# ototoi/pbrt-r3

Hardware: AMD Instinct MI355X
Metric: Mrays/s (higher is better)
Workload: dtype f32

## Files before the change

pbrt-r3_amd/csrc/pt_kernels.hip:

```cpp
#include <hip/hip_runtime.h>
#include <cstdlib>
#include "pt_device.h"
#include "pt_device_math.h"
#include "pt_bxdf.h"
#include "pt_sphere.h"
#include "pt_quadric.h"
#include "pt_texture.h"
#include <type_traits>
#include "pt_lobes.h"
#include "pt_kernels.h"
#include "../../include/pbrtgpu.h"

#if PT_QUADRIC
#define PT_KERNEL __global__
#ifndef PT_KERNEL_NS
#define PT_KERNEL_NS ptq
#endif
namespace PT_KERNEL_NS {
#else
#define PT_KERNEL extern "C" __global__
#endif

#ifndef PT_LIGHTS_IN_LDS
#define PT_LIGHTS_IN_LDS 8
// ... 717 lines not shown
PT_DEV float v_max3(float a, float b, float c) { float r; asm("v_max3_f32 %0, %1, %2, %3" : "=v"(r) : "v"(a), "v"(b), "v"(c)); return r; }
PT_DEV float v_min3(float a, float b, float c) { float r; asm("v_min3_f32 %0, %1, %2, %3" : "=v"(r) : "v"(a), "v"(b), "v"(c)); return r; }

template <bool EXACT>
PT_DEV void visit_node_general(const PtNode* nodes, uint32_t ni, V3 o, V3 idir, uint32_t sbits, float tmin, float tmax, TravCtx& c, uint32_t& top, uint32_t& sa) {
    const char* nb = reinterpret_cast<const char*>(nodes) + (size_t)(ni & PT_REF_INDEX_MASK) * 128u;
    const uint32_t ox = (sbits & 1u) ? 48u : 0u, oy = (sbits & 2u) ? 48u : 0u, oz = (sbits & 4u) ? 48u : 0u;
    float4 nx = *reinterpret_cast<const float4*>(nb + ox), fx = *reinterpret_cast<const float4*>(nb + (48u - ox));
    float4 ny = *reinterpret_cast<const float4*>(nb + 16u + oy), fy = *reinterpret_cast<const float4*>(nb + 16u + (48u - oy));
    float4 nz = *reinterpret_cast<const float4*>(nb + 32u + oz), fz = *reinterpret_cast<const float4*>(nb + 32u + (48u - oz));
    uint4 ch = *reinterpret_cast<const uint4*>(nb + 96u);
    uint32_t axes = *reinterpret_cast<const uint32_t*>(nb + 112u);
    uint32_t mask = 0;
#define PT_SLAB(k, C)                                                        \
    {                                                                        \
        float a = tmin, b = tmax;                                            \
        if (EXACT) {                                                         \
            a = sse_max(a, (nx.C - o.x) * idir.x); b = sse_min(b, (fx.C - o.x) * idir.x); \
            a = sse_max(a, (ny.C - o.y) * idir.y); b = sse_min(b, (fy.C - o.y) * idir.y); \
            a = sse_max(a, (nz.C - o.z) * idir.z); b = sse_min(b, (fz.C - o.z) * idir.z); \
        } else {                                                             \
            a = fmaxf(a, (nx.C - o.x) * idir.x); b = fminf(b, (fx.C - o.x) * idir.x); \
            a = fmaxf(a, (ny.C - o.y) * idir.y); b = fminf(b, (fy.C - o.y) * idir.y); \
            a = fmaxf(a, (nz.C - o.z) * idir.z); b = fminf(b, (fz.C - o.z) * idir.z); \
        }                                                                    \
        if (b >= a) mask |= (1u << k);                                       \
    }
    PT_SLAB(0, x) PT_SLAB(1, y) PT_SLAB(2, z) PT_SLAB(3, w)
#undef PT_SLAB
    mask &= (axes >> 8) & 15u;
    uint32_t s_top = (sbits >> (axes & 3)) & 1, s_left = (sbits >> ((axes >> 2) & 3)) & 1, s_right = (sbits >> ((axes >> 4) & 3)) & 1;
    uint32_t l0 = s_left ? ch.x : ch.y, l1 = s_left ? ch.y : ch.x;
    uint32_t l0b = s_left ? 1u : 2u, l1b = s_left ? 2u : 1u;
    uint32_t r0 = s_right ? ch.z : ch.w, r1 = s_right ? ch.w : ch.z;
    uint32_t r0b = s_right ? 4u : 8u, r1b = s_right ? 8u : 4u;
    uint32_t c0 = s_top ? l0 : r0, c1 = s_top ? l1 : r1, c2 = s_top ? r0 : l0, c3 = s_top ? r1 : l1;
    uint32_t b0 = s_top ? l0b : r0b, b1 = s_top ? l1b : r1b, b2 = s_top ? r0b : l0b, b3 = s_top ? r1b : l1b;
    if (mask & b0) fs_push(c, sa, top, c0);
    if (mask & b1) fs_push(c, sa, top, c1);
    if (mask & b2) fs_push(c, sa, top, c2);
    if (mask & b3) fs_push(c, sa, top, c3);
}
PT_DEV void node_step_general(const PtScene& sc, LaneRay& r, TravCtx& c) {
    const uint32_t ref = fs_pop(c, r.sa, r.top);
    c.n_nodes++;
    if (r.sbits & 8u) visit_node_general<true>(sc.nodes, ref, r.o, r.idir, r.sbits, r.tmin, r.tmax, c, r.top, r.sa);
    else visit_node_general<false>(sc.nodes, ref, r.o, r.idir, r.sbits, r.tmin, r.tmax, c, r.top, r.sa);
}
PT_DEV void fs_push4_exec(uint32_t& sa, uint32_t& top, uint32_t c0, uint32_t c1, uint32_t c2, uint32_t c3, unsigned long long e0, unsigned long long e1,
                          unsigned long long e2, unsigned long long e3) {
    unsigned long long sv;
    asm volatile(
        "s_mov_b64 %[sv], exec\n\t"
        "s_mov_b64 exec, %[e0]\n\t"
        "v_add_u32 %[sa], %[slot], %[sa]\n\t"
        "v_mov_b32 %[top], %[c0]\n\t"
        "ds_write_b32 %[sa], %[c0]\n\t"
        "s_mov_b64 exec, %[e1]\n\t"
        "v_add_u32 %[sa], %[slot], %[sa]\n\t"
        "v_mov_b32 %[top], %[c1]\n\t"
        "ds_write_b32 %[sa], %[c1]\n\t"
        "s_mov_b64 exec, %[e2]\n\t"
        "v_add_u32 %[sa], %[slot], %[sa]\n\t"
        "v_mov_b32 %[top], %[c2]\n\t"
        "ds_write_b32 %[sa], %[c2]\n\t"
        "s_mov_b64 exec, %[e3]\n\t"
        "v_add_u32 %[sa], %[slot], %[sa]\n\t"
        "v_mov_b32 %[top], %[c3]\n\t"
        "ds_write_b32 %[sa], %[c3]\n\t"
        "s_mov_b64 exec, %[sv]"
        : [sa] "+v"(sa), [top] "+v"(top), [sv] "=&s"(sv)
        : [e0] "s"(e0), [e1] "s"(e1), [e2] "s"(e2), [e3] "s"(e3), [c0] "v"(c0), [c1] "v"(c1), [c2] "v"(c2), [c3] "v"(c3), [slot] "s"(PT_SLOT)
        : "memory");
}
typedef float pt_v4f __attribute__((ext_vector_type(4)));
typedef uint32_t pt_v4u __attribute__((ext_vector_type(4)));
PT_DEV float4 lds_load4(uint32_t a) { const pt_v4f v = *(__attribute__((address_space(3))) const pt_v4f*)(size_t)a; return make_float4(v.x, v.y, v.z, v.w); }
PT_DEV uint4 lds_load4u(uint32_t a) { const pt_v4u v = *(__attribute__((address_space(3))) const pt_v4u*)(size_t)a; return make_uint4(v.x, v.y, v.z, v.w); }
PT_DEV void node_step_lean(const PtScene& sc, LaneRay& r, TravCtx& c) {
    const uint32_t ref = r.top;
    r.sa -= PT_SLOT;
    uint32_t top = lds_load(r.sa);
    c.n_nodes++;
    const char* nb = reinterpret_cast<const char*>(sc.nodes);
    const uint32_t no = ref << 7;
    float4 nx, fx, ny, fy, nz, fz;
    uint4 ch;
#if PT_TOP_NODES > 0
    const bool in_lds = no < c.top_bytes;
    c.n_nodes_lds += in_lds ? 1u : 0u;
    if (in_lds) {
        const uint32_t la = c.top_lds + no - (no >> 3);
        nx = lds_load4(la + r.o_nx); fx = lds_load4(la + r.o_fx); ny = lds_load4(la + r.o_ny); fy = lds_load4(la + r.o_fy);
        nz = lds_load4(la + r.o_nz); fz = lds_load4(la + r.o_fz);
        ch = lds_load4u(la + 96u);
    }
    if (!in_lds)
#endif
    {
        nx = *reinterpret_cast<const float4*>(nb + (no + r.o_nx)); fx = *reinterpret_cast<const float4*>(nb + (no + r.o_fx));
        ny = *reinterpret_cast<const float4*>(nb + (no + r.o_ny)); fy = *reinterpret_cast<const float4*>(nb + (no + r.o_fy));
        nz = *reinterpret_cast<const float4*>(nb + (no + r.o_nz)); fz = *reinterpret_cast<const float4*>(nb + (no + r.o_fz));
        ch = *reinterpret_cast<const uint4*>(nb + (no + 96u));
    }
    const float ox = r.o.x, oy = r.o.y, oz = r.o.z, ix = r.idir.x, iy = r.idir.y, iz = r.idir.z;
#define PT_SLAB(C) (v_min3(v_min(r.tmax, (fx.C - ox) * ix), (fy.C - oy) * iy, (fz.C - oz) * iz) >= v_max3(v_max(r.tmin, (nx.C - ox) * ix), (ny.C - oy) * iy, (nz.C - oz) * iz))
    const bool h0 = PT_SLAB(x), h1 = PT_SLAB(y), h2 = PT_SLAB(z), h3 = PT_SLAB(w);
#undef PT_SLAB
    const bool T = __builtin_amdgcn_ubfe(r.sbits, __builtin_amdgcn_ubfe(ch.x, PT_REF_AXIS_SHIFT, 2), 1) != 0u;
    const bool L = __builtin_amdgcn_ubfe(r.sbits, __builtin_amdgcn_ubfe(ch.y, PT_REF_AXIS_SHIFT, 2), 1) != 0u;
    const bool R = __builtin_amdgcn_ubfe(r.sbits, __builtin_amdgcn_ubfe(ch.w, PT_REF_AXIS_SHIFT, 2), 1) != 0u;
    const uint32_t l0 = L ? ch.x : ch.y, l1 = L ? ch.y : ch.x, r0 = R ? ch.z : ch.w, r1 = R ? ch.w : ch.z;
    const uint32_t c0 = T ? l0 : r0, c1 = T ? l1 : r1, c2 = T ? r0 : l0, c3 = T ? r1 : l1;
    const unsigned long long H0 = __ballot(h0), H1 = __ballot(h1), H2 = __ballot(h2), H3 = __ballot(h3), Tm = __ballot(T), Lm = __ballot(L), Rm = __ballot(R);
    const unsigned long long yl = Lm & (H0 ^ H1), el0 = H1 ^ yl, el1 = H0 ^ yl;
    const unsigned long long yr = Rm & (H2 ^ H3), er0 = H3 ^ yr, er1 = H2 ^ yr;
    const unsigned long long y0 = Tm & (el0 ^ er0), e0 = er0 ^ y0, e2 = el0 ^ y0;
    const unsigned long long y1 = Tm & (el1 ^ er1), e1 = er1 ^ y1, e3 = el1 ^ y1;
    fs_push4_exec(r.sa, top, c0, c1, c2, c3, e0, e1, e2, e3);
    r.top = top;
}

#define PT_PAIR_U(x) ((uint32_t)__builtin_amdgcn_update_dpp(0, (int)(x), 0xB1, 0xF, 0xF, false))
#define PT_PAIR_F(x) __builtin_bit_cast(float, __builtin_amdgcn_update_dpp(0, __builtin_bit_cast(int, (x)), 0xB1, 0xF, 0xF, false))
PT_DEV void node_step_coop(const PtScene& sc, LaneRay& r, TravCtx& c, bool w_node, unsigned long long m_node) {
    constexpr unsigned long long kEven = 0x5555555555555555ull, kOdd = 0xAAAAAAAAAAAAAAAAull;
    const unsigned long long ev = m_node & kEven, od = m_node & kOdd;
    const unsigned long long m_y = ev | (ev << 1), m_z = od | (od >> 1);
    if (__builtin_amdgcn_inverse_ballot_w64(m_y | m_z)) {
        const uint32_t ref = r.top;
        const uint32_t no = ref << 7;
        const char* nb = reinterpret_cast<const char*>(sc.nodes);
        uint32_t top = PT_EMPTY_REF;
        const bool in_lds = w_node && no < c.top_bytes;
        if (w_node) { r.sa -= PT_SLOT; top = lds_load(r.sa); c.n_nodes++; c.n_nodes_lds += in_lds ? 1u : 0u; }
        const unsigned long long m_lds = __ballot(in_lds), le = m_lds & kEven, lo = m_lds & kOdd;
        const unsigned long long y_lds = le | (le << 1), z_lds = lo | (lo >> 1);
        const uint32_t base = in_lds ? c.top_lds + no - (no >> 3) : no;
        uint32_t a1 = base + r.o_nx, a2 = base + r.o_ny, a3 = base + r.o_nz;
        uint32_t b1 = PT_PAIR_U(base + r.o_fx), b2 = PT_PAIR_U(base + r.o_fy), b3 = PT_PAIR_U(base + r.o_fz);
        unsigned long long sv;
        asm volatile("s_mov_b64 %[sv], exec\n\ts_and_b64 exec, exec, %[om]\n\tv_swap_b32 %0, %3\n\tv_swap_b32 %1, %4\n\tv_swap_b32 %2, %5\n\ts_mov_b64 exec, %[sv]"
                     : "+v"(a1), "+v"(a2), "+v"(a3), "+v"(b1), "+v"(b2), "+v"(b3), [sv] "=&s"(sv) : [om] "s"(kOdd));
        float4 x1, x2, x3, x4, x5, x6;
        uint4 ch;
        if (__builtin_amdgcn_inverse_ballot_w64(m_y & y_lds)) { x1 = lds_load4(a1); x2 = lds_load4(a2); x3 = lds_load4(a3); }
        if (__builtin_amdgcn_inverse_ballot_w64(m_z & z_lds)) { x4 = lds_load4(b1); x5 = lds_load4(b2); x6 = lds_load4(b3); }
        if (in_lds) ch = lds_load4u(base + 96u);
        if (__builtin_amdgcn_inverse_ballot_w64(m_y & ~y_lds)) {
            x1 = *reinterpret_cast<const float4*>(nb + a1); x2 = *reinterpret_cast<const float4*>(nb + a2); x3 = *reinterpret_cast<const float4*>(nb + a3);
        }
        if (__builtin_amdgcn_inverse_ballot_w64(m_z & ~z_lds)) {
            x4 = *reinterpret_cast<const float4*>(nb + b1); x5 = *reinterpret_cast<const float4*>(nb + b2); x6 = *reinterpret_cast<const float4*>(nb + b3);
        }
        if (__builtin_amdgcn_inverse_ballot_w64(m_node & ~m_lds)) ch = *reinterpret_cast<const uint4*>(nb + (no + 96u));
        asm volatile("s_mov_b64 %[sv], exec\n\ts_and_b64 exec, exec, %[om]\n\t"
                     "v_swap_b32 %0, %12\n\tv_swap_b32 %1, %13\n\tv_swap_b32 %2, %14\n\tv_swap_b32 %3, %15\n\t"
                     "v_swap_b32 %4, %16\n\tv_swap_b32 %5, %17\n\tv_swap_b32 %6, %18\n\tv_swap_b32 %7, %19\n\t"
                     "v_swap_b32 %8, %20\n\tv_swap_b32 %9, %21\n\tv_swap_b32 %10, %22\n\tv_swap_b32 %11, %23\n\t"
                     "s_mov_b64 exec, %[sv]\n\ts_nop 1"
                     : "+v"(x1.x), "+v"(x1.y), "+v"(x1.z), "+v"(x1.w), "+v"(x2.x), "+v"(x2.y), "+v"(x2.z), "+v"(x2.w), "+v"(x3.x), "+v"(x3.y), "+v"(x3.z), "+v"(x3.w),
                       "+v"(x4.x), "+v"(x4.y), "+v"(x4.z), "+v"(x4.w), "+v"(x5.x), "+v"(x5.y), "+v"(x5.z), "+v"(x5.w), "+v"(x6.x), "+v"(x6.y), "+v"(x6.z), "+v"(x6.w), [sv] "=&s"(sv)
                     : [om] "s"(kOdd));
        const float ox = r.o.x, oy = r.o.y, oz = r.o.z, ix = r.idir.x, iy = r.idir.y, iz = r.idir.z;
#define PT_SLAB(C) (v_min3(v_min(r.tmax, (PT_PAIR_F(x4.C) - ox) * ix), (PT_PAIR_F(x5.C) - oy) * iy, (PT_PAIR_F(x6.C) - oz) * iz) >= \
                    v_max3(v_max(r.tmin, (x1.C - ox) * ix), (x2.C - oy) * iy, (x3.C - oz) * iz))
        const bool h0 = PT_SLAB(x), h1 = PT_SLAB(y), h2 = PT_SLAB(z), h3 = PT_SLAB(w);
#undef PT_SLAB
        const bool T = __builtin_amdgcn_ubfe(r.sbits, __builtin_amdgcn_ubfe(ch.x, PT_REF_AXIS_SHIFT, 2), 1) != 0u;
        const bool L = __builtin_amdgcn_ubfe(r.sbits, __builtin_amdgcn_ubfe(ch.y, PT_REF_AXIS_SHIFT, 2), 1) != 0u;
        const bool R = __builtin_amdgcn_ubfe(r.sbits, __builtin_amdgcn_ubfe(ch.w, PT_REF_AXIS_SHIFT, 2), 1) != 0u;
        const uint32_t l0 = L ? ch.x : ch.y, l1 = L ? ch.y : ch.x, r0 = R ? ch.z : ch.w, r1 = R ? ch.w : ch.z;
        const uint32_t c0 = T ? l0 : r0, c1 = T ? l1 : r1, c2 = T ? r0 : l0, c3 = T ? r1 : l1;
        const unsigned long long H0 = __ballot(h0) & m_node, H1 = __ballot(h1) & m_node, H2 = __ballot(h2) & m_node, H3 = __ballot(h3) & m_node;
        const unsigned long long Tm = __ballot(T), Lm = __ballot(L), Rm = __ballot(R);
        const unsigned long long yl = Lm & (H0 ^ H1), el0 = H1 ^ yl, el1 = H0 ^ yl;
        const unsigned long long yr = Rm & (H2 ^ H3), er0 = H3 ^ yr, er1 = H2 ^ yr;
        const unsigned long long y0 = Tm & (el0 ^ er0), e0 = er0 ^ y0, e2 = el0 ^ y0;
        const unsigned long long y1 = Tm & (el1 ^ er1), e1 = er1 ^ y1, e3 = el1 ^ y1;
        fs_push4_exec(r.sa, top, c0, c1, c2, c3, e0, e1, e2, e3);
        if (w_node) r.top = top;
    }
}

template <bool SPH, bool INST, bool ALPHA = false>
PT_DEV int32_t trace_closest(const PtScene& sc, V3 o, V3 d, float t_max, TravCtx& c, float* t_out, uint32_t* inst_out) {
// ... 48 lines not shown
        PREFETCH = 14, HANDOUT = 15,
        ITERATIONS = 16, HANDOUTS = 17, HANDOUTS_CLK = 18,
        EMPTY = 19, EMPTY_CLK = 20,
        SLOTS = 24
    };
    unsigned long long slot[SLOTS];
    long long t_start, t_iter, t_mark;
    bool handout;
    static PT_DEV long long now() { return (long long)__builtin_readcyclecounter(); }
    PT_DEV void start() { for (int i = 0; i < SLOTS; i++) slot[i] = 0; t_start = now(); }
    PT_DEV void iteration() {
        t_iter = now();
        handout = false;
        if ((slot[ITERATIONS]++ & 63ull) == 0ull) {
            const long long e0 = now();
            const long long e1 = now();
            slot[EMPTY] += 1; slot[EMPTY_CLK] += (unsigned long long)(e1 - e0);
            t_iter = now();
        }
        t_mark = t_iter;
    }
    PT_DEV void mark() { t_mark = now(); }
    PT_DEV void lap(int s) { const long long t = now(); slot[s] += (unsigned long long)(t - t_mark); t_mark = t; }
    PT_DEV void hand_out() { handout = true; }
    PT_DEV void handed_out() {
        const unsigned long long dt = (unsigned long long)(now() - t_mark);
        slot[HANDOUT] += dt;
        if (handout) { slot[HANDOUTS] += 1; slot[HANDOUTS_CLK] += dt; }
    }
    PT_DEV void serviced() { t_mark = now(); slot[SERVICE] += (unsigned long long)(t_mark - t_iter); }
    PT_DEV void round(int clk, int rounds, int items, unsigned long long n) { lap(clk); slot[rounds] += 1; slot[items] += n; }
    PT_DEV void node_round(unsigned long long lanes) { round(NODE, NODE_ROUNDS, NODE_LANES, (unsigned long long)__popcll(lanes)); }
    PT_DEV void general_round(unsigned long long lanes) { round(GENERAL, GENERAL_ROUNDS, NODE_LANES, (unsigned long long)__popcll(lanes)); }
    PT_DEV void leaf_round(unsigned long long items) { round(LEAF_FINISH, LEAF_ROUNDS, LEAF_ITEMS, items); }
    PT_DEV void leaf_issued() { lap(LEAF_ISSUE); asm volatile("s_waitcnt vmcnt(0)" ::: "memory"); lap(LEAF_WAIT); }
    PT_DEV void finish(uint32_t* diag, uint32_t lane) {
        slot[TOTAL] = (unsigned long long)(now() - t_start);
        if (lane == 0) for (int i = 0; i < SLOTS; i++) atomicAdd(reinterpret_cast<unsigned long long*>(diag) + i, slot[i]);
    }
};
#else
#define PT_PROF_BEGIN() ((void)0)
#define PT_PROF(call) ((void)0)
#endif
#ifndef PT_REFILL_MIN
#define PT_REFILL_MIN 8
#endif
#ifndef PT_LEAF_MIN
#define PT_LEAF_MIN 24
#endif
#ifndef PT_LEAF_MIN_INST
#define PT_LEAF_MIN_INST 40
#endif
#ifndef PT_TRACE_WAVES
#define PT_TRACE_WAVES 4
#endif
#ifndef PT_TRACE_DIST_WAVES
#define PT_TRACE_DIST_WAVES 4
#endif

#ifndef PT_LEAF_LANES_MIN
#define PT_LEAF_LANES_MIN 18
#endif
static_assert(PT_LEAF_LANES_MIN > 0, "the leaf round is triggered by the number of parked lanes");
#ifndef PT_SPH_LANES_MIN
#define PT_SPH_LANES_MIN 8
#endif
PT_DEV uint32_t wave_max_scan(uint32_t x) {
    x = max(x, (uint32_t)__builtin_amdgcn_update_dpp(0, (int)x, 0x111, 0xf, 0xf, false));
    x = max(x, (uint32_t)__builtin_amdgcn_update_dpp(0, (int)x, 0x112, 0xf, 0xf, false));
    x = max(x, (uint32_t)__builtin_amdgcn_update_dpp(0, (int)x, 0x114, 0xf, 0xf, false));
    x = max(x, (uint32_t)__builtin_amdgcn_update_dpp(0, (int)x, 0x118, 0xf, 0xf, false));
    x = max(x, (uint32_t)__builtin_amdgcn_update_dpp(0, (int)x, 0x142, 0xa, 0xf, false));
    x = max(x, (uint32_t)__builtin_amdgcn_update_dpp(0, (int)x, 0x143, 0xc, 0xf, false));
    return x;
}
template <bool DIST, bool SPH, bool INST = false, bool FAR = false, bool ALPHA = false>
PT_DEV void trace_body(const PtScene& sc, const PtPaths& P, const PtQueues& Q, PtCounters* cnt, uint32_t* spill, uint32_t spill_depth, uint32_t* err) {
    constexpr uint32_t TB = DIST ? PT_TBLOCK : PT_BLOCK;
    __shared__ uint32_t s_stack[(DIST ? PT_FS_SLOTS : PT_LDS_STACK) * TB];
    __shared__ unsigned long long s_cnt[4];
    __shared__ float4 s_res[DIST ? TB : 1];
#if PT_TOP_NODES > 0
    __shared__ float4 s_top[DIST ? PT_TOP_NODES * 7 : 1];
#endif
    TravCtx c;
    c.lds = &s_stack[threadIdx.x];
    c.top_lds = 0; c.top_bytes = 0; c.n_nodes_lds = 0;
    c.spill_stride = gridDim.x * TB;
    c.spill = spill + PT_DIAG_WORDS + (size_t)blockIdx.x * TB + threadIdx.x;
    c.spill_depth = spill_depth;
    c.n_nodes = 0; c.n_tris = 0; c.overflow = 0;
    c.lane_base = 0; c.stage_wave = 0; c.stage_own = 0; c.idx_pub = 0; c.idx_ld = 0;
    if constexpr (DIST) {
        s_stack[threadIdx.x] = PT_EMPTY_REF;
        c.lane_base = lds_addr_of(&s_stack[threadIdx.x]);
    }
#if PT_TOP_NODES > 0
    if constexpr (DIST) {
        const uint32_t n_top = min(sc.n_top, (uint32_t)PT_TOP_NODES);
        const float4* src = reinterpret_cast<const float4*>(sc.nodes);
        for (uint32_t k = threadIdx.x; k < n_top * 7u; k += TB) { const uint32_t nd = k / 7u; s_top[k] = src[nd * 8u + (k - nd * 7u)]; }
        c.top_lds = lds_addr_of(reinterpret_cast<const uint32_t*>(s_top));
        c.top_bytes = n_top << 7;
        __syncthreads();
    }
#endif
    const uint32_t n_cur = Q.counts[PT_Q_CUR], n_sh = Q.counts[PT_Q_SHADOW], n_pr = Q.counts[PT_Q_PROBE];
    const uint32_t total = n_cur + n_sh + n_pr;
    const uint32_t lane = threadIdx.x & 63;
    const unsigned long long below = (lane == 0) ? 0ull : (~0ull >> (64 - lane));
    unsigned long long regular = 0, shadow = 0;

    int kind = 0;
    uint32_t p = 0;
    LaneRay r;
    r.sp = 0;
    r.sa = c.lane_base; r.sa_limit = 0;
    r.top = PT_EMPTY_REF;
    bool more = total > 0;
    bool sph_wait = false;
    int pf_stage = 0, pf_kind = 0;
    uint32_t pf_raw = 0, pf_count = 0, pf_used = 0, pf_p = 0;
    uint32_t seg = blockIdx.x & 7u, seg_dry = 0;
    const uint32_t seg_len = (((total + 7u) >> 3) + 63u) & ~63u;
    float4 pf_o = make_float4(0.0f, 0.0f, 0.0f, 0.0f), pf_d = pf_o;
    PT_PROF_BEGIN();
    for (;;) {
        PT_PROF(iteration());
        constexpr bool PF_BYPASS = DIST && !FAR;
        int pf_gate = pf_stage;
        if constexpr (PF_BYPASS) asm volatile("" : "+s"(pf_gate));
        if (PF_BYPASS && pf_gate == 3) {
        } else if (pf_stage == 0) {
            if (more) {
                if (lane == 0) pf_raw = atomicAdd(&Q.counts[PT_Q_SEG_TICKET0 + 32u * seg], 64u);
                pf_stage = 1;
            }
        } else if (pf_stage == 1) {
            const uint32_t seg_lo = seg * seg_len, seg_hi = min(total, seg_lo + seg_len);
            const uint32_t base = seg_lo + (uint32_t)__builtin_amdgcn_readfirstlane((int)pf_raw);
            if (seg_lo >= total || base >= seg_hi) {
                seg = (seg + 1u) & 7u;
                if (++seg_dry == 8u) more = false;
                pf_stage = 0;
            } else {
                seg_dry = 0;
                pf_count = min(64u, seg_hi - base);
                pf_used = 0;
                const uint32_t item = base + lane;
                if (lane < pf_count) {
                    if (item < n_cur) { pf_p = Q.cur[item]; pf_kind = 1; }
                    else if (item < n_cur + n_sh) { pf_p = Q.shadow[item - n_cur]; pf_kind = 2; }
                    else { pf_p = Q.probe[item - n_cur - n_sh]; pf_kind = 3; }
                }
                pf_stage = 2;
            }
        } else if (pf_stage == 2) {
            if (lane < pf_count) {
                const float4* so = pf_kind == 1 ? P.ray_o : (pf_kind == 2 ? P.sh_o : P.pr_o);
                const float4* sd = pf_kind == 1 ? P.ray_d : (pf_kind == 2 ? P.sh_d : P.pr_d);
                pf_o = so[pf_p]; pf_d = sd[pf_p];
            }
            pf_stage = 3;
        }
        PT_PROF(lap(PhaseProf::PREFETCH));
        constexpr bool LATE_RETIRE = DIST;
#define PT_RETIRE()                                                                                                                                      \
        if (kind != 0 && ray_done(r)) {                                                                                                                  \
            if (kind == 1) { P.hit_t[p] = r.ray_tmax; P.hit_rec[p] = r.best; if (INST && (!ALPHA || sc.n_instances)) P.hit_inst[p] = r.best_inst; }      \
            else if (kind == 2) P.occluded[p] = r.best >= 0 ? 1 : 0;                                                                                     \
            else P.probe_rec[p] = r.best;                                                                                                                \
            kind = 0;                                                                                                                                    \
        }
        if constexpr (LATE_RETIRE) {
            if (!more) { PT_RETIRE() }
        } else {
            PT_RETIRE()
        }
        {
            const unsigned long long idle = LATE_RETIRE ? __ballot(kind == 0 || ray_done(r)) : __ballot(kind == 0);
            const uint32_t n_idle = (uint32_t)__popcll(idle);
            if (pf_stage == 3 && (n_idle >= PT_REFILL_MIN || idle == ~0ull || (!more && n_idle != 0))) {
                PT_PROF(hand_out());
                if constexpr (LATE_RETIRE) { PT_RETIRE() }
                const uint32_t take = min(n_idle, pf_count - pf_used);
                const uint32_t rank = (uint32_t)__popcll(idle & below);
                const int src = (int)((pf_used + rank) & 63u);
                const uint32_t np = (uint32_t)__shfl((int)pf_p, src, 64);
                const int nk = __shfl(pf_kind, src, 64);
                float4 ro, rd;
                ro.x = __shfl(pf_o.x, src, 64); ro.y = __shfl(pf_o.y, src, 64); ro.z = __shfl(pf_o.z, src, 64); ro.w = __shfl(pf_o.w, src, 64);
                rd.x = __shfl(pf_d.x, src, 64); rd.y = __shfl(pf_d.y, src, 64); rd.z = __shfl(pf_d.z, src, 64);
                if (kind == 0 && rank < take) {
                    p = np; kind = nk;
                    if (nk == 2) shadow++; else regular++;
                    if constexpr (DIST) ray_begin_fs(sc, r, c, f4_3(ro), mk3(rd.x, rd.y, rd.z), ro.w);
                    else ray_begin(sc, r, f4_3(ro), mk3(rd.x, rd.y, rd.z), ro.w);
                }
                pf_used += take;
                if (pf_used == pf_count) pf_stage = 0;
            }
        }
#undef PT_RETIRE
        PT_PROF(handed_out());
        if ((LATE_RETIRE ? __ballot(kind != 0 && !ray_done(r)) : __ballot(kind != 0)) == 0) {
            if (!more && pf_stage == 0) break;
            continue;
        }
        bool w_tri = kind != 0 && ray_wants_tri(r);
        bool w_node = kind != 0 && ray_wants_node(r);
        unsigned long long m_tri = __ballot(w_tri), m_node = __ballot(w_node);
        PT_PROF(serviced());
        if constexpr (DIST) {
            bool sround = false;
            unsigned long long m_tri_s = 0;
            if constexpr (SPH) {
                m_tri_s = __ballot(w_tri && sph_wait);
                m_tri &= ~m_tri_s;
            }
            const bool sph_go = SPH && (uint32_t)__popcll(m_tri_s) >= (uint32_t)PT_SPH_LANES_MIN;
            const uint32_t tcnt = w_tri ? ((r.top >> PT_LEAF_COUNT_SHIFT) & 7u) + 1u : 0u;
            uint32_t tcnt_r = tcnt;
            bool w_serve = w_tri;
            constexpr uint32_t LEAF_DUE = 56u;
            unsigned long long c0 = 0, c1 = 0, c2 = 0, c3 = 0;
            const uint32_t leaf_level = (sph_go || (uint32_t)__popcll(m_tri) >= (uint32_t)PT_LEAF_LANES_MIN) ? LEAF_DUE : 0u;
            const uint32_t wbase = threadIdx.x & ~63u;
            constexpr bool HACC = !SPH;
            uint32_t lf_pre = 0, lf_items = 0;
            bool lf_served = false, lf_valid = false;
            int lf_kk = 0;
            float lf_tmax = PT_INF;
            RayPre lf_rp;
            TriVerts lf_tv;
            auto leaf_issue = [&](auto sr_tag) {
                constexpr bool SR = decltype(sr_tag)::value;
                (void)SR;
                c0 = __ballot((tcnt_r & 1u) != 0); c1 = __ballot((tcnt_r & 2u) != 0); c2 = __ballot((tcnt_r & 4u) != 0); c3 = __ballot((tcnt_r & 8u) != 0);
                lf_pre = (uint32_t)(__popcll(c0 & below) + 2 * __popcll(c1 & below) + 4 * __popcll(c2 & below) + 8 * __popcll(c3 & below));
                lf_served = w_serve && lf_pre + tcnt_r <= 64u;
                const unsigned long long m_served = __ballot(lf_served);
                const int last = 63 - __clzll(m_served);
                lf_items = (uint32_t)__shfl((int)(lf_pre + tcnt_r), last, 64);
                typedef uint32_t __attribute__((may_alias)) map_word;
                map_word* const s_own = reinterpret_cast<map_word*>(&s_res[wbase]);
                s_own[lane] = 0u;
                if (lf_served) s_own[lf_pre] = ((lf_pre << 6) | lane) + 1u;
                __builtin_amdgcn_fence(__ATOMIC_RELEASE, "wavefront");
                __builtin_amdgcn_wave_barrier();
                __builtin_amdgcn_fence(__ATOMIC_ACQUIRE, "wavefront");
                lf_valid = lane < lf_items;
                const uint32_t own_w = wave_max_scan(s_own[lane]) - 1u;
                const int o = (int)(own_w & 63u);
                const uint32_t k = lane - (own_w >> 6);
                const uint32_t first = (uint32_t)__shfl((int)(r.top & PT_LEAF_FIRST_MASK), o, 64);
                lf_rp.o = mk3(__shfl(r.rp.o.x, o, 64), __shfl(r.rp.o.y, o, 64), __shfl(r.rp.o.z, o, 64));
                lf_rp.d = mk3(0.0f, 0.0f, 0.0f);
                if ((SPH && SR) || sc.any_one_sided) lf_rp.d = mk3(__shfl(r.rp.d.x, o, 64), __shfl(r.rp.d.y, o, 64), __shfl(r.rp.d.z, o, 64));
                if constexpr ((SPH && SR) || HACC) lf_tmax = __shfl(r.ray_tmax, o, 64);
                lf_kk = __shfl(r.rp.kx | (r.rp.ky << 2) | (r.rp.kz << 4) | ((kind == 2 ? 1 : 0) << 6), o, 64);
                lf_rp.kx = lf_kk & 3; lf_rp.ky = (lf_kk >> 2) & 3; lf_rp.kz = (lf_kk >> 4) & 3;
                lf_rp.sx = __shfl(r.rp.sx, o, 64); lf_rp.sy = __shfl(r.rp.sy, o, 64); lf_rp.sz = __shfl(r.rp.sz, o, 64);
                lf_rp.dperm = lf_rp.d;
                lf_tv.p0 = lf_rp.d; lf_tv.p1 = lf_rp.d; lf_tv.p2 = lf_rp.d; lf_tv.prim = 0; lf_tv.flags = 0;
                if (lf_valid) lf_tv = load_tri(sc.tris, first + k);
            };
            auto leaf_finish = [&](auto sr_tag) {
                constexpr bool SR = decltype(sr_tag)::value;
                (void)SR;
                bool sphere_rec = false;
                if constexpr (SPH) sphere_rec = lf_valid && (lf_tv.flags & PT_TRI_SPHERE) != 0;
                unsigned long long m_sitems = 0;
                if constexpr (SPH && !SR) { m_sitems = __ballot(sphere_rec); }
                bool cand = false;
                if (lf_valid) {
                    asm("" : "+v"(lf_tv.p0.x), "+v"(lf_tv.p0.y), "+v"(lf_tv.p0.z), "+v"(lf_tv.p1.x), "+v"(lf_tv.p1.y), "+v"(lf_tv.p1.z), "+v"(lf_tv.p2.x), "+v"(lf_tv.p2.y), "+v"(lf_tv.p2.z));
                    TriCore tc;
                    const bool tri_ok = tri_core(lf_rp, lf_tv.p0, lf_tv.p1, lf_tv.p2, lf_tv.flags, tc);
                    float4 res = make_float4(tri_ok ? 1.0f : 0.0f, tc.t_scaled, tc.det, tc.t);
                    if constexpr (HACC) cand = tri_ok && tri_accept(tc.t_scaled, tc.det, lf_tmax);
                    if (SR && sphere_rec) {
                        SphHit sh;
                        sh.t = 0.0f; sh.a_hi = 0.0f; sh.b_hi = 0.0f;
                        const bool ok = shape_hit_test_inl(sc.spheres[__float_as_uint(lf_tv.p0.x)], lf_rp.o, lf_rp.d, lf_tmax, (lf_kk & 64) ? 2.0f * PT_PI : PT_PI, &sh);
                        res = make_float4(ok ? 2.0f : 0.0f, sh.a_hi, sh.b_hi, sh.t);
                        cand = ok;
                    }
                    if (!HACC || cand) s_res[wbase + lane] = res;
                }
                const unsigned long long m_cand = HACC ? __ballot(cand) : 0ull;
                (void)m_cand;
                __builtin_amdgcn_fence(__ATOMIC_RELEASE, "wavefront");
                __builtin_amdgcn_wave_barrier();
                __builtin_amdgcn_fence(__ATOMIC_ACQUIRE, "wavefront");
                bool walk = lf_served;
                if constexpr (SPH) {
                    if (!SR && lf_served && ((m_sitems >> lf_pre) & ((1ull << tcnt_r) - 1ull)) != 0ull) { sph_wait = true; walk = false; }
                    if (SR && lf_served) sph_wait = false;
                }
                if (walk) {
                    const uint32_t rec0 = fs_pop(c, r.sa, r.top) & PT_LEAF_FIRST_MASK;
                    const bool any_hit = kind == 2;
                    bool leaf_hit = false;
                    uint32_t tested = tcnt;
                    if constexpr (HACC) {
                    uint32_t bits = (uint32_t)(m_cand >> lf_pre) & ((1u << tcnt) - 1u);
                    bool first = true;
                    while (bits != 0u) {
                        const uint32_t k = (uint32_t)__builtin_ctz(bits);
                        bits &= bits - 1u;
                        const float4 v = s_res[wbase + lf_pre + k];
                        bool acc;
                        if (SPH && SR && v.x == 2.0f) acc = !(v.y > r.ray_tmax) && !(v.z > r.ray_tmax);
                        else acc = first || tri_accept(v.y, v.z, r.ray_tmax);
                        first = false;
                        if (acc) {
                            r.best = (int32_t)(rec0 + k); leaf_hit = true;
                            if (any_hit) { r.sa = c.lane_base; r.top = PT_EMPTY_REF; tested = k + 1u; break; }
                            r.ray_tmax = v.w;
                        }
                    }
                    } else {
                    bool stop = false;
                    for (uint32_t k0 = 0; k0 < tcnt && !stop; k0 += 4u) {
                        const uint32_t b = wbase + lf_pre + k0;
                        const float4 va = s_res[b], vb = s_res[wbase + min(lf_pre + k0 + 1u, 63u)], vc = s_res[wbase + min(lf_pre + k0 + 2u, 63u)],
                                     vd = s_res[wbase + min(lf_pre + k0 + 3u, 63u)];
                        auto step = [&](const float4 v, uint32_t k) {
                            if (stop || k >= tcnt) return;
                            bool acc;
                            if (SPH && SR && v.x == 2.0f) acc = !(v.y > r.ray_tmax) && !(v.z > r.ray_tmax);
                            else acc = v.x != 0.0f && tri_accept(v.y, v.z, r.ray_tmax);
                            if (acc) {
                                r.best = (int32_t)(rec0 + k); leaf_hit = true;
                                if (any_hit) { r.sa = c.lane_base; r.top = PT_EMPTY_REF; tested = k + 1; stop = true; return; }
                                r.ray_tmax = v.w;
                            }
                        };
                        step(va, k0); step(vb, k0 + 1u); step(vc, k0 + 2u); step(vd, k0 + 3u);
                    }
                    }
                    c.n_tris += tested;
                    if (leaf_hit && !any_hit) r.tmax = r.ray_tmax;
                }
            };
            const bool lean = __ballot(w_node && r.sa >= r.sa_limit) == 0ull;
            if (lean && m_node != 0 && leaf_level < LEAF_DUE) {
                PT_PROF(mark());
                if constexpr (FAR) node_step_coop(sc, r, c, w_node, m_node);
                else if (w_node) node_step_lean(sc, r, c);
                PT_PROF(node_round(m_node));
            } else if (m_node != 0 && leaf_level < LEAF_DUE) {
                PT_PROF(mark());
                if (w_node) node_step_general(sc, r, c);
                PT_PROF(general_round(m_node));
            } else if ((m_tri | m_tri_s) != 0) {
                if constexpr (SPH) {
                    sround = sph_go || m_tri == 0;
                    w_serve = w_tri && (sph_wait == sround);
                    tcnt_r = w_serve ? tcnt : 0u;
                }
                PT_PROF(mark());
                if (SPH && sround) leaf_issue(std::true_type{}); else leaf_issue(std::false_type{});
                PT_PROF(leaf_issued());
                if (SPH && sround) leaf_finish(std::true_type{}); else leaf_finish(std::false_type{});
                PT_PROF(leaf_round(lf_items));
            }
        } else {
        if (m_node != 0 && __popcll(m_tri) < (INST ? PT_LEAF_MIN_INST : PT_LEAF_MIN)) {
            if (w_node) ray_step_node(sc, r, c);
            PT_PROF(general_round(m_node));
        } else {
            if constexpr (INST) {
                if (w_tri) {
                    if (r.top == PT_INST_EXIT_REF) {
                        (void)stk_pop(c, r.top, r.sp);
                        const float w_tmax = __uint_as_float(stk_pop(c, r.top, r.sp)), w_tmin = __uint_as_float(stk_pop(c, r.top, r.sp));
                        const float4 ro = (kind == 1 ? P.ray_o : (kind == 2 ? P.sh_o : P.pr_o))[p], rd = (kind == 1 ? P.ray_d : (kind == 2 ? P.sh_d : P.pr_d))[p];
                        const bool hit_inside = r.best >= 0 && r.best_inst == r.cur_inst;
                        ray_set_direction_state(r, f4_3(ro), mk3(rd.x, rd.y, rd.z));
                        r.tmin = w_tmin; r.tmax = hit_inside ? r.ray_tmax : w_tmax;
                        r.cur_inst = 0;
                    } else ray_step_tri_enter<SPH, ALPHA>(sc, r, kind == 2, c);
                }
            } else {
                if (w_tri) ray_step_tri<SPH, INST>(sc, r, kind == 2, c);
            }
            PT_PROF(leaf_round((unsigned long long)__popcll(m_tri)));
        }
        }
    }
    PT_PROF(finish(spill, lane));
    if (c.overflow) atomicOr(err, 1u);
    flush_counters(cnt, s_cnt, regular, shadow, c.n_nodes, c.n_tris);
    {
        unsigned long long v = c.n_nodes_lds;
        for (int o = 32; o > 0; o >>= 1) v += (unsigned long long)__shfl_xor((int)(v >> 32), o, 64) << 32 | (unsigned int)__shfl_xor((int)(unsigned int)v, o, 64);
        if ((threadIdx.x & 63) == 0 && v) atomicAdd(&cnt->nodes_lds, v);
    }
}
PT_KERNEL void __launch_bounds__(PT_TBLOCK, PT_TRACE_DIST_WAVES) k_trace(PtScene sc, PtPaths P, PtQueues Q, PtCounters* cnt, uint32_t* spill,
                                                              uint32_t spill_depth, uint32_t* err) {
    trace_body<true, false>(sc, P, Q, cnt, spill, spill_depth, err);
}
PT_KERNEL void __launch_bounds__(PT_TBLOCK, PT_TRACE_DIST_WAVES) k_trace_far(PtScene sc, PtPaths P, PtQueues Q, PtCounters* cnt, uint32_t* spill,
                                                                   uint32_t spill_depth, uint32_t* err) {
    trace_body<true, false, false, true>(sc, P, Q, cnt, spill, spill_depth, err);
}
PT_KERNEL void __launch_bounds__(PT_BLOCK, PT_TRACE_WAVES) k_trace_seq(PtScene sc, PtPaths P, PtQueues Q, PtCounters* cnt, uint32_t* spill,
                                                                  uint32_t spill_depth, uint32_t* err) {
    trace_body<false, false>(sc, P, Q, cnt, spill, spill_depth, err);
}
#ifndef PT_TRACE_INST_WAVES
#define PT_TRACE_INST_WAVES 3
#endif

PT_KERNEL void __launch_bounds__(PT_BLOCK, PT_TRACE_INST_WAVES) k_trace_inst(PtScene sc, PtPaths P, PtQueues Q, PtCounters* cnt, uint32_t* spill,
                                                                       uint32_t spill_depth, uint32_t* err) {
    trace_body<false, true, true>(sc, P, Q, cnt, spill, spill_depth, err);
}
PT_KERNEL void __launch_bounds__(PT_BLOCK, PT_TRACE_INST_WAVES) k_trace_alpha(PtScene sc, PtPaths P, PtQueues Q, PtCounters* cnt, uint32_t* spill,
                                                                        uint32_t spill_depth, uint32_t* err) {
    trace_body<false, true, true, false, true>(sc, P, Q, cnt, spill, spill_depth, err);
}
PT_KERNEL void __launch_bounds__(PT_TBLOCK, PT_TRACE_DIST_WAVES) k_trace_sph_dist(PtScene sc, PtPaths P, PtQueues Q, PtCounters* cnt, uint32_t* spill,
                                                                           uint32_t spill_depth, uint32_t* err) {
    trace_body<true, true>(sc, P, Q, cnt, spill, spill_depth, err);
}
PT_KERNEL void __launch_bounds__(PT_BLOCK, 2) k_trace_sph(PtScene sc, PtPaths P, PtQueues Q, PtCounters* cnt, uint32_t* spill,
// ... 2998 lines not shown
```

pbrt-r3_amd/csrc/pt_scene_upload.cpp:

```cpp
#include "pt_context_impl.h"

namespace {

bool load_sobol(pt_context* ctx) {
    std::string path = ctx->data_dir + "/sobol_tables.bin";
    FILE* f = std::fopen(path.c_str(), "rb");
    if (!f) return false;
    char magic[8];
    uint32_t hdr[4];
    bool ok = std::fread(magic, 1, 8, f) == 8 && std::memcmp(magic, "PTSOBOL1", 8) == 0 && std::fread(hdr, 4, 4, f) == 4;
    if (ok) {
        ctx->sobol_msize = hdr[1];
        ctx->sobol_n_vdc = hdr[2];
        ctx->sobol_n_inv = hdr[3];
        ctx->sobol_m32.resize((size_t)hdr[0] * hdr[1]);
        ctx->sobol_vdc.resize((size_t)hdr[2] * hdr[1]);
        ctx->sobol_inv.resize((size_t)hdr[3] * hdr[1]);
        ok = std::fread(ctx->sobol_m32.data(), 4, ctx->sobol_m32.size(), f) == ctx->sobol_m32.size() &&
             std::fread(ctx->sobol_vdc.data(), 8, ctx->sobol_vdc.size(), f) == ctx->sobol_vdc.size() &&
             std::fread(ctx->sobol_inv.data(), 8, ctx->sobol_inv.size(), f) == ctx->sobol_inv.size();
    }
    std::fclose(f);
    return ok;
}
// ... 1149 lines not shown
    return PT_OK;
}

pt_status upload_images_and_textures(pt_context* ctx, const pt_scene_desc* d, const SceneChecks& chk, const MaterialTables& mt, bool& images_on_device) {
    pt_status st;
    std::vector<PtImage> dimages(d->n_images);
    images_on_device =(mt.any_textured || !ctx->inf_lights.empty() || !ctx->map_lights.empty() || mt.any_alpha_tex) && d->n_images;
    if (images_on_device) {
        size_t total = 0;
        for (uint32_t i = 0; i < d->n_images; i++) {
            const pt_image& im = d->images[i];
            PtImage& o = dimages[i];
            std::memset(&o, 0, sizeof(o));
            o.width = im.width; o.height = im.height; o.channels = im.channels; o.n_levels = im.n_levels;
            uint32_t w = im.width, h = im.height;
            size_t off = 0;
            for (uint32_t l = 0; l < im.n_levels; l++) {
                if (off > 0xffffffffull) return ctx->fail(PT_ERR_UNSUPPORTED, "image pyramid larger than 2^32 floats");
                o.level_off[l] = (uint32_t)off;
                off += (size_t)w * h * im.channels;
                if (w > 1) w /= 2;
                if (h > 1) h /= 2;
            }
            total += off;
        }
        std::vector<float> all(total);
        size_t at = 0;
        std::vector<size_t> base(d->n_images);
        for (uint32_t i = 0; i < d->n_images; i++) {
            size_t n = 0;
            uint32_t w = d->images[i].width, h = d->images[i].height;
            for (uint32_t l = 0; l < d->images[i].n_levels; l++) { n += (size_t)w * h * d->images[i].channels; if (w > 1) w /= 2; if (h > 1) h /= 2; }
            std::memcpy(all.data() + at, d->images[i].texels, n * sizeof(float));
            base[i] = at;
            at += n;
        }
        if ((st = upload(ctx, ctx->d_image_texels, all.data(), all.size())) != PT_OK) return st;
        for (uint32_t i = 0; i < d->n_images; i++) dimages[i].texels = ctx->d_image_texels.as<float>() + base[i];
        if ((st = upload(ctx, ctx->d_images, dimages.data(), dimages.size())) != PT_OK) return st;
    } else { ctx->d_image_texels.release(); ctx->d_images.release(); }
    if (mt.any_textured || chk.any_alpha) {
        if (d->n_textures) { if ((st = upload(ctx, ctx->d_textures, d->textures, d->n_textures)) != PT_OK) return st; } else ctx->d_textures.release();
        if ((st = upload(ctx, ctx->d_tex_prog, mt.tex_prog.data(), mt.tex_prog.size())) != PT_OK) return st;
    } else { ctx->d_textures.release(); ctx->d_tex_prog.release(); }
    if (mt.any_textured) { if ((st = upload(ctx, ctx->d_mat_params, mt.mparams.data(), mt.mparams.size())) != PT_OK) return st; } else ctx->d_mat_params.release();
    if (d->N) { if ((st = upload(ctx, ctx->d_N, d->N, 3 * (size_t)d->n_vertices)) != PT_OK) return st; } else ctx->d_N.release();
    if (d->S) { if ((st = upload(ctx, ctx->d_S, d->S, 3 * (size_t)d->n_vertices)) != PT_OK) return st; } else ctx->d_S.release();
    if (d->UV) { if ((st = upload(ctx, ctx->d_UV, d->UV, 2 * (size_t)d->n_vertices)) != PT_OK) return st; } else ctx->d_UV.release();
    return PT_OK;
}

void fill_scene_record(pt_context* ctx, const pt_scene_desc* d, const SceneChecks& chk, const MaterialTables& mt, const WorldBuild& w, bool images_on_device) {
    PtScene& sc = ctx->sc;
    sc.nodes = ctx->d_nodes.as<PtNode>();
    sc.tris = ctx->d_tris.as<PtTri>();
    sc.tri_info = ctx->d_tri_info.as<PtTriInfo>();
    sc.N = d->N ? ctx->d_N.as<float>() : nullptr;
    sc.S = d->S ? ctx->d_S.as<float>() : nullptr;
    sc.UV = d->UV ? ctx->d_UV.as<float>() : nullptr;
    sc.materials = ctx->d_materials.as<PtMaterial>();
    sc.general_materials = mt.general_materials ? 1u : 0u;
    ctx->scene_has_lobe_materials = mt.general_materials;
    sc.any_one_sided = w.any_one_sided ? 1u : 0u;
    sc.dist_leaves = (w.up_max_leaf <= 8 && !std::getenv("PBRTGPU_SEQ_LEAVES")) ? 1u : 0u;
    ctx->n_materials = d->n_materials;
    sc.lights = ctx->d_lights.as<PtLight>();
    sc.n_lights = (uint32_t)w.lights.size();
    sc.textured = mt.any_textured ? 1u : 0u;
    sc.textures = (mt.any_textured || chk.any_alpha) && d->n_textures ? ctx->d_textures.as<pt_texture>() : nullptr;
    sc.tex_prog = (mt.any_textured || chk.any_alpha) ? ctx->d_tex_prog.as<uint32_t>() : nullptr;
    ctx->scene_alpha = chk.any_alpha;
    ctx->quadric_kernels = false;
    for (uint32_t i = 0; i < d->n_spheres; i++) ctx->quadric_kernels |= d->spheres[i].kind != PT_SHAPE_SPHERE;
    sc.images = images_on_device ? ctx->d_images.as<PtImage>() : nullptr;
    sc.mat_params = mt.any_textured ? ctx->d_mat_params.as<PtMatParams>() : nullptr;
    sc.spheres = d->n_spheres ? ctx->d_spheres.as<PtSphere>() : nullptr;
    sc.instances = d->n_instances ? ctx->d_instances.as<PtInstance>() : nullptr;
    sc.n_instances = d->n_instances;
    sc.n_spheres = d->n_spheres;
    if (d->n_spheres) sc.general_materials = 1;
    if (d->n_instances) { sc.general_materials = 1; sc.dist_leaves = 0; }
    sc.general_materials = (sc.general_materials & 1u) | ((uint32_t)mt.mixes.size() << 1);
    sc.root_ref = w.up_root_ref;
    sc.n_top = w.n_top;
    for (int a = 0; a < 3; a++) { const float ext = w.up_root_hi[a] - w.up_root_lo[a]; sc.cell_scale[a] = ext > 0.0f ? (float)(1u << PT_SORT_CELL_BITS) / ext : 0.0f; }
    std::memcpy(sc.wb_min, w.up_root_lo, 12);
    std::memcpy(sc.wb_max, w.up_root_hi, 12);
}

pt_status build_delta_and_env_records(pt_context* ctx, const pt_scene_desc* d, const std::vector<PtLight>& lights, std::vector<float>& env_power, std::vector<float>& delta_power) {
    PtScene& sc = ctx->sc;
    pt_status st;
    env_power.assign(ctx->inf_lights.size(), 0.0f);
    delta_power.assign(ctx->delta_lights.size() + ctx->map_lights.size(), 0.0f);
    sc.n_envs = 0;
    sc.n_deltas = 0;
    std::vector<PtEnvLight> envs(ctx->inf_lights.size());
    std::vector<PtDeltaLight> deltas(ctx->delta_lights.size() + ctx->map_lights.size());
    std::vector<PtMapLight> maps(ctx->map_lights.size());
    ctx->maplight_kernels = !ctx->map_lights.empty();
    const float dx = sc.wb_max[0] - sc.wb_min[0], dy = sc.wb_max[1] - sc.wb_min[1], dz = sc.wb_max[2] - sc.wb_min[2];
    const float radius = std::sqrt(dx * dx + dy * dy + dz * dz) * 0.5f;
    if (!ctx->delta_lights.empty()) {
        const float kPiF = 3.14159265358979323846f;
        auto lum = [](float r, float g, float b) { return 0.212671f * r + 0.715160f * g + 0.072169f * b; };
        for (size_t k = 0; k < ctx->delta_lights.size(); k++) {
            const pt_delta_light& dl = ctx->delta_lights[k];
            PtDeltaLight& o = deltas[k];
            std::memset(&o, 0, sizeof(o));
            o.kind = (uint32_t)dl.kind;
            std::memcpy(o.spectrum, dl.spectrum, 12);
            const float* m = dl.light_to_world;
            float s = 0.0f;
            if (dl.kind == PT_DELTA_DISTANT) {
                const float x = dl.direction[0], y = dl.direction[1], z = dl.direction[2];
                const float vx = m[0] * x + m[1] * y + m[2] * z, vy = m[4] * x + m[5] * y + m[6] * z, vz = m[8] * x + m[9] * y + m[10] * z;
                const float len = std::sqrt(vx * vx + vy * vy + vz * vz);
                o.v[0] = vx / len; o.v[1] = vy / len; o.v[2] = vz / len;
                o.radius = radius;
                s = kPiF * radius * radius;
            } else {
                for (int a = 0; a < 3; a++) o.v[a] = m[4 * a] * 0.0f + m[4 * a + 1] * 0.0f + m[4 * a + 2] * 0.0f + m[4 * a + 3];
                if (dl.kind == PT_DELTA_SPOT) {
                    o.cos_total_width = std::cos(dl.cone_total_width * (kPiF / 180.0f));
                    o.cos_falloff_start = std::cos(dl.cone_falloff_start * (kPiF / 180.0f));
                    for (int a = 0; a < 3; a++)
                        for (int b = 0; b < 3; b++) o.w2l[3 * a + b] = dl.world_to_light[4 * a + b];
                    s = 2.0f * kPiF * (1.0f - 0.5f * (o.cos_falloff_start - o.cos_total_width));
                } else {
                    s = 4.0f * kPiF;
                }
            }
            delta_power[k] = lum(o.spectrum[0] * s, o.spectrum[1] * s, o.spectrum[2] * s);
        }
    }
    for (size_t k = 0; k < maps.size(); k++) {
        const pt_map_light& ml = ctx->map_lights[k];
        PtDeltaLight& o = deltas[ctx->delta_lights.size() + k];
        PtMapLight& mo = maps[k];
        std::memset(&o, 0, sizeof(o));
        std::memset(&mo, 0, sizeof(mo));
        o.kind = (uint32_t)ml.kind;
        o.pad = (uint32_t)k;
        std::memcpy(o.spectrum, ml.spectrum, 12);
        const float* m = ml.light_to_world;
        for (int a = 0; a < 3; a++) o.v[a] = m[4 * a] * 0.0f + m[4 * a + 1] * 0.0f + m[4 * a + 2] * 0.0f + m[4 * a + 3];
        std::memcpy(mo.w2l, ml.world_to_light, 48);
        mo.image = (uint32_t)ml.image;
        const EnvMap map(d->images[ml.image]);
        float c[3];
        map.lookup(0.5f, 0.5f, 0.5f, c);
        const float kPiF = 3.14159265358979323846f;
        float pw[3];
        if (ml.kind == PT_DELTA_GONIOMETRIC) {
            for (int a = 0; a < 3; a++) pw[a] = 4.0f * kPiF * o.spectrum[a] * c[a];
        } else {
            const float aspect = (float)ml.resolution[0] / (float)ml.resolution[1];
            if (aspect > 1.0f) { mo.screen[0] = -aspect; mo.screen[1] = -1.0f; mo.screen[2] = aspect; mo.screen[3] = 1.0f; }
            else { mo.screen[0] = -1.0f; mo.screen[1] = -1.0f / aspect; mo.screen[2] = 1.0f; mo.screen[3] = 1.0f / aspect; }
            pth::Xf proj;
            if (!pth::xf_perspective(ml.fov, 1e-3f, 1e30f, &proj)) return ctx->fail(PT_ERR_INVALID_ARGUMENT, "projection light: fov gives a singular projection");
            std::memcpy(mo.proj, proj.m.a, 64);
            const float* q = proj.inv.a;
            const float x = mo.screen[2], y = mo.screen[3], z = 0.0f;
            float cx = q[0] * x + q[1] * y + q[2] * z + q[3], cy = q[4] * x + q[5] * y + q[6] * z + q[7], cz = q[8] * x + q[9] * y + q[10] * z + q[11];
            const float cw = q[12] * x + q[13] * y + q[14] * z + q[15];
            if (cw != 1.0f) { cx = cx / cw; cy = cy / cw; cz = cz / cw; }
// ... 394 lines not shown
```

Baseline: 1198.

## Store top BVH nodes unpacked in LDS and simplify traversal lane-state ballots

For the non-FAR path, top-level nodes are copied into LDS at their full 128-byte stride. The LDS base is folded into the node offset so LDS and global loads share one address computation and the per-node packed-address arithmetic goes away. Lane classification ballots are rewritten to test the stack-top reference directly, and compiler barriers keep the popcounts scalar. The LDS footprint grows by one eighth, and the top-node cache is disabled for very large BVHs so offset arithmetic cannot overflow the 32-bit range.

```diff
diff --git a/pbrt-r3_amd/csrc/pt_kernels.hip b/pbrt-r3_amd/csrc/pt_kernels.hip
--- a/pbrt-r3_amd/csrc/pt_kernels.hip
+++ b/pbrt-r3_amd/csrc/pt_kernels.hip
@@ -823,26 +823,22 @@
     r.sa -= PT_SLOT;
     uint32_t top = lds_load(r.sa);
     c.n_nodes++;
-    const char* nb = reinterpret_cast<const char*>(sc.nodes);
-    const uint32_t no = ref << 7;
     float4 nx, fx, ny, fy, nz, fz;
     uint4 ch;
-#if PT_TOP_NODES > 0
+    const uint32_t no = (ref << 7) + c.top_lds;
+    const char* nb = reinterpret_cast<const char*>(sc.nodes) - c.top_lds;
+    const uint32_t a_nx = no + r.o_nx, a_fx = no + r.o_fx, a_ny = no + r.o_ny, a_fy = no + r.o_fy, a_nz = no + r.o_nz, a_fz = no + r.o_fz;
     const bool in_lds = no < c.top_bytes;
     c.n_nodes_lds += in_lds ? 1u : 0u;
     if (in_lds) {
-        const uint32_t la = c.top_lds + no - (no >> 3);
-        nx = lds_load4(la + r.o_nx); fx = lds_load4(la + r.o_fx); ny = lds_load4(la + r.o_ny); fy = lds_load4(la + r.o_fy);
-        nz = lds_load4(la + r.o_nz); fz = lds_load4(la + r.o_fz);
-        ch = lds_load4u(la + 96u);
-    }
-    if (!in_lds)
-#endif
-    {
-        nx = *reinterpret_cast<const float4*>(nb + (no + r.o_nx)); fx = *reinterpret_cast<const float4*>(nb + (no + r.o_fx));
-        ny = *reinterpret_cast<const float4*>(nb + (no + r.o_ny)); fy = *reinterpret_cast<const float4*>(nb + (no + r.o_fy));
-        nz = *reinterpret_cast<const float4*>(nb + (no + r.o_nz)); fz = *reinterpret_cast<const float4*>(nb + (no + r.o_fz));
-        ch = *reinterpret_cast<const uint4*>(nb + (no + 96u));
+        nx = lds_load4(a_nx); fx = lds_load4(a_fx); ny = lds_load4(a_ny); fy = lds_load4(a_fy); nz = lds_load4(a_nz); fz = lds_load4(a_fz);
+        ch = lds_load4u(no + 96u);
+    }
+    if (!in_lds) {
+        nx = *reinterpret_cast<const float4*>(nb + a_nx); fx = *reinterpret_cast<const float4*>(nb + a_fx);
+        ny = *reinterpret_cast<const float4*>(nb + a_ny); fy = *reinterpret_cast<const float4*>(nb + a_fy);
+        nz = *reinterpret_cast<const float4*>(nb + a_nz); fz = *reinterpret_cast<const float4*>(nb + a_fz);
+        ch = *reinterpret_cast<const uint4*>(nb + (size_t)no + 96u);
     }
     const float ox = r.o.x, oy = r.o.y, oz = r.o.z, ix = r.idir.x, iy = r.idir.y, iz = r.idir.z;
 #define PT_SLAB(C) (v_min3(v_min(r.tmax, (fx.C - ox) * ix), (fy.C - oy) * iy, (fz.C - oz) * iz) >= v_max3(v_max(r.tmin, (nx.C - ox) * ix), (ny.C - oy) * iy, (nz.C - oz) * iz))
@@ -1057,7 +1053,7 @@
     __shared__ unsigned long long s_cnt[4];
     __shared__ float4 s_res[DIST ? TB : 1];
 #if PT_TOP_NODES > 0
-    __shared__ float4 s_top[DIST ? PT_TOP_NODES * 7 : 1];
+    __shared__ float4 s_top[DIST ? PT_TOP_NODES * 8 : 1];
 #endif
     TravCtx c;
     c.lds = &s_stack[threadIdx.x];
@@ -1075,9 +1071,15 @@
     if constexpr (DIST) {
         const uint32_t n_top = min(sc.n_top, (uint32_t)PT_TOP_NODES);
         const float4* src = reinterpret_cast<const float4*>(sc.nodes);
-        for (uint32_t k = threadIdx.x; k < n_top * 7u; k += TB) { const uint32_t nd = k / 7u; s_top[k] = src[nd * 8u + (k - nd * 7u)]; }
-        c.top_lds = lds_addr_of(reinterpret_cast<const uint32_t*>(s_top));
-        c.top_bytes = n_top << 7;
+        if constexpr (FAR) {
+            for (uint32_t k = threadIdx.x; k < n_top * 7u; k += TB) { const uint32_t nd = k / 7u; s_top[k] = src[nd * 8u + (k - nd * 7u)]; }
+            c.top_lds = lds_addr_of(reinterpret_cast<const uint32_t*>(s_top));
+            c.top_bytes = n_top << 7;
+        } else {
+            for (uint32_t k = threadIdx.x; k < n_top * 8u; k += TB) s_top[k] = src[k];
+            c.top_lds = n_top ? lds_addr_of(reinterpret_cast<const uint32_t*>(s_top)) : 0u;
+            c.top_bytes = c.top_lds + (n_top << 7);
+        }
         __syncthreads();
     }
 #endif
@@ -1154,7 +1156,9 @@
             PT_RETIRE()
         }
         {
-            const unsigned long long idle = LATE_RETIRE ? __ballot(kind == 0 || ray_done(r)) : __ballot(kind == 0);
+            uint32_t top_now = r.top;
+            if constexpr (LATE_RETIRE) asm("" : "+v"(top_now));
+            const unsigned long long idle = LATE_RETIRE ? __ballot(top_now == PT_EMPTY_REF) : __ballot(kind == 0);
             const uint32_t n_idle = (uint32_t)__popcll(idle);
             if (pf_stage == 3 && (n_idle >= PT_REFILL_MIN || idle == ~0ull || (!more && n_idle != 0))) {
                 PT_PROF(hand_out());
@@ -1179,28 +1183,32 @@
         }
 #undef PT_RETIRE
         PT_PROF(handed_out());
-        if ((LATE_RETIRE ? __ballot(kind != 0 && !ray_done(r)) : __ballot(kind != 0)) == 0) {
+        if ((LATE_RETIRE ? __ballot(!ray_done(r)) : __ballot(kind != 0)) == 0) {
             if (!more && pf_stage == 0) break;
             continue;
         }
-        bool w_tri = kind != 0 && ray_wants_tri(r);
-        bool w_node = kind != 0 && ray_wants_node(r);
+        bool w_tri = (int32_t)r.top < -1;
+        bool w_node = (int32_t)r.top >= 0;
         unsigned long long m_tri = __ballot(w_tri), m_node = __ballot(w_node);
         PT_PROF(serviced());
         if constexpr (DIST) {
             bool sround = false;
             unsigned long long m_tri_s = 0;
             if constexpr (SPH) {
-                m_tri_s = __ballot(w_tri && sph_wait);
+                m_tri_s = __ballot(sph_wait) & m_tri;
                 m_tri &= ~m_tri_s;
             }
-            const bool sph_go = SPH && (uint32_t)__popcll(m_tri_s) >= (uint32_t)PT_SPH_LANES_MIN;
+            uint32_t n_sph = (uint32_t)__popcll(m_tri_s);
+            if constexpr (SPH) asm("" : "+s"(n_sph));
+            const bool sph_go = SPH && n_sph >= (uint32_t)PT_SPH_LANES_MIN;
             const uint32_t tcnt = w_tri ? ((r.top >> PT_LEAF_COUNT_SHIFT) & 7u) + 1u : 0u;
             uint32_t tcnt_r = tcnt;
             bool w_serve = w_tri;
             constexpr uint32_t LEAF_DUE = 56u;
             unsigned long long c0 = 0, c1 = 0, c2 = 0, c3 = 0;
-            const uint32_t leaf_level = (sph_go || (uint32_t)__popcll(m_tri) >= (uint32_t)PT_LEAF_LANES_MIN) ? LEAF_DUE : 0u;
+            uint32_t n_parked = (uint32_t)__popcll(m_tri);
+            asm("" : "+s"(n_parked));
+            const uint32_t leaf_level = (sph_go || n_parked >= (uint32_t)PT_LEAF_LANES_MIN) ? LEAF_DUE : 0u;
             const uint32_t wbase = threadIdx.x & ~63u;
             constexpr bool HACC = !SPH;
             uint32_t lf_pre = 0, lf_items = 0;
@@ -1320,7 +1328,7 @@
                     if (leaf_hit && !any_hit) r.tmax = r.ray_tmax;
                 }
             };
-            const bool lean = __ballot(w_node && r.sa >= r.sa_limit) == 0ull;
+            const bool lean = (__ballot(r.sa >= r.sa_limit) & m_node) == 0ull;
             if (lean && m_node != 0 && leaf_level < LEAF_DUE) {
                 PT_PROF(mark());
                 if constexpr (FAR) node_step_coop(sc, r, c, w_node, m_node);
diff --git a/pbrt-r3_amd/csrc/pt_scene_upload.cpp b/pbrt-r3_amd/csrc/pt_scene_upload.cpp
--- a/pbrt-r3_amd/csrc/pt_scene_upload.cpp
+++ b/pbrt-r3_amd/csrc/pt_scene_upload.cpp
@@ -1255,7 +1255,7 @@
     if (d->n_instances) { sc.general_materials = 1; sc.dist_leaves = 0; }
     sc.general_materials = (sc.general_materials & 1u) | ((uint32_t)mt.mixes.size() << 1);
     sc.root_ref = w.up_root_ref;
-    sc.n_top = w.n_top;
+    sc.n_top = w.up_n_nodes > (size_t)(1u << 25) - 1280u ? 0u : w.n_top;
     for (int a = 0; a < 3; a++) { const float ext = w.up_root_hi[a] - w.up_root_lo[a]; sc.cell_scale[a] = ext > 0.0f ? (float)(1u << PT_SORT_CELL_BITS) / ext : 0.0f; }
     std::memcpy(sc.wb_min, w.up_root_lo, 12);
     std::memcpy(sc.wb_max, w.up_root_hi, 12);
```

New measurement: 1206 (median of 6 runs). No clear change (+0.7%).
